# alexfreudenberg/miraculix

Measured on AMD Instinct MI355X. Metric: effective GFLOP/s for dgemm_compressed (2-bit SNP x fp64), higher is better.
Workload: dtype f64; 1 GPU; 1000000x50000 (SNPs x indiv), ncol=32, dgemm_compressed N+T per step, uncentred; snps=1000000, indiv=50000, ncol=32, parallelism=snp-shard1, form=one process per GPU

## Files before the change

include/miraculix_amd.h:

```cpp
#ifndef MIRACULIX_AMD_H
#define MIRACULIX_AMD_H

#include <stdbool.h>
#include <stddef.h>
#include <stdint.h>

#ifdef __cplusplus
extern "C" {
#endif
#if defined(__GNUC__)
#pragma GCC visibility push(default)
#endif


void setOptions_compressed(int use_gpu, int cores, int floatLoop, int meanSubstract, int ignore_missings,
                           int do_not_center, int do_normalize, int use_miraculix_freq, int variant,
                           int print_details);

void plink2compressed(char *plink, char *plink_transposed, int snps, int indiv, double *f, int max_n,
                      void **compressed);

void dgemm_compressed(char *trans, void *compressed, int n, double *B, int Ldb, double *C, int Ldc);

void free_compressed(void **compressed);
// ... 62 lines not shown
} mxa_multi_info;
typedef struct mxa_shard_info {
  int device; long snp_begin, snp_end;
  int peer_to_root, peer_from_root;
  int kernel_launches; double kernel_ms;
  int in_copies; double in_ms;
  int out_copies; double out_ms;
  int pushes; double push_ms;
} mxa_shard_info;
int mxa_multi_get_info(void *compressed, mxa_multi_info *out);
int mxa_multi_shard_info(void *compressed, int shard, mxa_shard_info *out);
int mxa_multi_reset_profile(void *compressed);

int mxa_snp_multiply_panel(const unsigned char *snp_matrix, int snps, int indiv, int col_begin, int col_end, int upper_only,
                           double *panel, long ld, int is_plink_format);

int mxa_grm(const unsigned char *plink_transposed, int snps, int indiv, double *G, int is_plink_format, int do_scale,
            const double *allele_freq);
int mxa_ld(const unsigned char *plink, int snps, int indiv, double *R, int is_plink_format, const double *allele_freq);

int mxa_ld_band(const unsigned char *plink, int snps, int indiv, int window, double *band, long ldb, int kind, int is_plink_format,
                const double *allele_freq);
int mxa_ld_scores(const unsigned char *plink, int snps, int indiv, int window, double *scores, int adjust, int is_plink_format,
                  const double *allele_freq);

int mxa_ld_band_pairwise(const unsigned char *plink, int snps, int indiv, int window, double *band, long ldb, int kind);
int mxa_ld_scores_pairwise(const unsigned char *plink, int snps, int indiv, int window, double *scores, int adjust);

int mxa_set_engine(int engine);
int mxa_get_engine(void);
int mxa_last_path(void);
int mxa_last_range_fallback(void *compressed);

void mxa_profile_reset(void);
void mxa_profile_get(int *launches, double *total_ms);

void mxa_last_geometry(long *m, long *k, int *n, int *splits, int *a_tile, int *c_tile);
long mxa_plan_partial_doubles(long m, long k, int n);
int mxa_single_orientation(void *compressed);
long mxa_partial_capacity(void *compressed);

#if defined(__GNUC__)
#pragma GCC visibility pop
#endif
#ifdef __cplusplus
}
#endif
#endif
```

miraculix_amd/csrc/mxa_api.cpp:

```cpp
#include "../../include/miraculix_amd.h"
#include "mxa_internal.h"

#include <algorithm>
#include <atomic>
#include <chrono>
#include <cstdarg>
#include <cstdio>
#include <cstdlib>
#include <cstring>
#include <mutex>
#include <string>
#include <vector>

namespace mxa {

static int g_err = 0;
static char g_errmsg[512] = "";

Options &options() { static Options o; return o; }
Profile &profile() { static Profile p; return p; }
Geometry &last_geometry() { static Geometry g; return g; }
static bool g_profile_on = true;
static std::atomic<int> g_engine{[] {
  const char *e = getenv("MXA_ENGINE");
// ... 695 lines not shown
  const bool use_lut = n <= 2 && !no_plain;
  GemmPlan p = use_lut ? plan_lut(m, G.k_pad, n) : plan_gemm(m, G.k_pad, n);
  int splits_per_group = p.splits;
  if (!use_lut) {
    const size_t one = (size_t)p.n_pad * p.m_pad, need = one * p.splits;
    const size_t budget = partial_budget(w, need, one);
    if (budget < need) {
      splits_per_group = (int)std::max<size_t>(1, budget / one);
      GemmPlan pg = p; pg.splits = splits_per_group;
      if (ensure_partials(w, pg, s)) return 1;
    }
  }
  if (splits_per_group == p.splits && ensure_partials(w, p, s)) return 1;
  clock_mark("partials");
  {
    std::lock_guard<std::mutex> lk(g_prof_mutex);
    Geometry &geo = last_geometry();
    geo.m = m; geo.k = k; geo.n = n; geo.splits = p.splits; geo.a = p.a; geo.c = p.c; geo.path = use_lut ? 1 : 0;
  }
  const bool tr = !use_lut && gemm_use_tr(p, h, trans);
  const PackedMatrix &GL = gemm_operand(h, trans, tr);
  int mode = gemm_default_mode(p.c);
  const int *d_E = nullptr;
  if (!use_lut && (mode == 2 || mode == 3)) {
    if (w.cap_exp < (size_t)n) {
      MXA_HIP(hipStreamSynchronize(s));
      if (w.d_exp) { MXA_HIP(hipFree(w.d_exp)); w.d_exp = nullptr; w.cap_exp = 0; }
      MXA_HIP(hipMalloc(reinterpret_cast<void **>(&w.d_exp), sizeof(int) * (size_t)n));
      w.cap_exp = n;
    }
    if (launch_colexp(dB, ldb, k, n, w.d_colpart, w.d_exp, 0, s, w.d_denflag, kDenMaxSpan, -100000)) return 1;
    d_E = w.d_exp;
  }
  if (!use_lut && launch_pack_B(dB, ldb, k, n, w.d_Bp, G.k_pad, p.n_pad, p.c, s, d_E, 0, -1, nullptr, mode == 3 && !tr)) return 1;
  if (prof) MXA_HIP(hipEventRecord(pe0, s));
  if (splits_per_group < p.splits) {
    const size_t stride = (size_t)p.n_pad * p.m_pad;
    for (int pass = 0; pass < (d_E ? 2 : 1); pass++) {
      const int *gate = pass ? w.d_denflag : nullptr;
      if (pass && launch_pack_B(dB, ldb, k, n, w.d_Bp, G.k_pad, p.n_pad, p.c, s, nullptr, 0, -1, gate)) return 1;
      for (int sb = 0; sb < p.splits; sb += splits_per_group) {
        const int se = std::min(p.splits, sb + splits_per_group);
        if ((size_t)(se - sb) * stride > w.cap_P) { set_error(4, "internal: a group of %d K splits exceeds the partial-sum workspace", se - sb); return 1; }
        if (launch_gemm(GL, w.d_Bp, w.d_P, p, pass ? 0 : mode, s, next_ctr(w), sb, se, gate, tr, sb)) return 1;
        const int group = (sb > 0 ? 1 : 0) | (se < p.splits ? 2 : 0);
        if (launch_finish(w.d_P, p, m, n, dC, ldc, fill_rows, trans ? 1 : 0, centered, d_sumB, d_sumfB, h->d_f, s, pass ? nullptr : d_E, 0, 0, gate, nullptr, se - sb, group)) return 1;
      }
      if (!pass && prof) { MXA_HIP(hipEventRecord(pe1, s)); h->prof_pending[slot] = true; }
    }
    return 0;
  }
  int rc = use_lut ? launch_lut(G, dB, ldb, n, w.d_P, p, s) : launch_gemm(GL, w.d_Bp, w.d_P, p, mode, s, next_ctr(w), 0, -1, nullptr, tr);
  if (prof && !rc) { MXA_HIP(hipEventRecord(pe1, s)); h->prof_pending[slot] = true; }
  if (!rc && d_E) {
    rc = launch_pack_B(dB, ldb, k, n, w.d_Bp, G.k_pad, p.n_pad, p.c, s, nullptr, 0, -1, w.d_denflag);
    if (!rc) rc = launch_gemm(GL, w.d_Bp, w.d_P, p, 0, s, next_ctr(w), 0, -1, w.d_denflag, tr);
  }
  if (!rc) rc = launch_finish(w.d_P, p, m, n, dC, ldc, fill_rows, trans ? 1 : 0, centered, d_sumB, d_sumfB, h->d_f, s, d_E, 0, 0, nullptr, d_E ? w.d_denflag : nullptr);
  return rc;
}


constexpr int kPipeChunks = 8;
static const size_t kPipeMinBytes = (size_t)32 << 20;

static int pipe_setup(Handle *h) {
  for (hipStream_t &ps : h->pipe) if (!ps) MXA_HIP(hipStreamCreateWithFlags(&ps, hipStreamNonBlocking));
  for (hipEvent_t &e : h->pev) if (!e) MXA_HIP(hipEventCreateWithFlags(&e, hipEventDisableTiming));
  return 0;
}

static int gemm_host_pipelined(Handle *h, bool trans, int n, const double *B, long ldb, bool b_host, bool b_local, double *C, long ldc, bool c_host, bool c_local,
                               long fill_rows) {
  const int engine = g_engine.load();
  if ((engine != 0 && engine != 3) || n < 3 || getenv("MXA_DIAG")) return 2;
  if (engine == 0 && n <= kSmallNMaxColsHost) return 2;
  const PackedMatrix &G = trans ? h->snp_major : h->ind_major;
  const long m = G.rows, k = G.k;
  const size_t b_bytes = b_host ? sizeof(double) * (size_t)k * n : 0, c_bytes = c_host ? sizeof(double) * (size_t)m * n : 0;
  if (std::max(b_bytes, c_bytes) < kPipeMinBytes) return 2;
  const bool kmode = b_bytes >= c_bytes;
  const bool centered = options().centered;
  if (centered && !h->has_f) { set_error(6, "dgemm_compressed: centring requested but no allele frequencies were supplied to plink2compressed"); return 1; }
  if (n > h->max_n) h->max_n = n;
  if (ensure_workspace(h, n) || pipe_setup(h)) return 1;
  harvest_profile(h);
  Workspace &w = h->ws;
  hipStream_t s = h->stream;
  if (grow(&w.d_colpart, &w.cap_colpart, (size_t)n * (128 * (kPipeChunks + 1) + 2) + 16)) return 1;
// ... 501 lines not shown
int mxa_set_engine(int engine) {
  if (engine != 0 && engine != 1 && engine != 3 && engine != 4) return g_engine.load();
  return g_engine.exchange(engine);
}
int mxa_get_engine(void) { return g_engine.load(); }

void mxa_profile_reset(void) { profile() = Profile(); }
void mxa_profile_get(int *launches, double *total_ms) {
  if (launches) *launches = profile().launches;
  if (total_ms) *total_ms = profile().total_ms;
}
int mxa_last_path(void) {
  Geometry g;
  { std::lock_guard<std::mutex> lk(g_prof_mutex); g = last_geometry(); }
  if (g.path != 4) return g.path;
  int flag = 0, prev = 0;
  if (!g.d_flag) return 2;
  (void)hipGetDevice(&prev);
  if (hipSetDevice(g.flag_dev) != hipSuccess || hipMemcpy(&flag, g.d_flag, sizeof(int), hipMemcpyDeviceToHost) != hipSuccess) { (void)hipGetLastError(); flag = 0; }
  (void)hipSetDevice(prev);
  return flag ? 3 : 2;
}
int mxa_last_range_fallback(void *compressed) {
  if (!compressed || is_multi(compressed)) return -1;
  Handle *h = as_handle(compressed, "mxa_last_range_fallback");
  if (!h || !h->ws.d_denflag) return -1;
  int flag = 0, prev = 0;
  (void)hipGetDevice(&prev);
  if (hipSetDevice(h->device) != hipSuccess || hipStreamSynchronize(h->stream) != hipSuccess ||
      hipMemcpy(&flag, h->ws.d_denflag, sizeof(int), hipMemcpyDeviceToHost) != hipSuccess) { (void)hipGetLastError(); flag = -1; }
  (void)hipSetDevice(prev);
  return flag;
}
void mxa_last_geometry(long *m, long *k, int *n, int *splits, int *a_tile, int *c_tile) {
  const Geometry &g = last_geometry();
  if (m) *m = g.m; if (k) *k = g.k; if (n) *n = g.n; if (splits) *splits = g.splits; if (a_tile) *a_tile = g.a; if (c_tile) *c_tile = g.c;
}

long mxa_plan_partial_doubles(long m, long k, int n) {
  if (m <= 0 || k <= 0 || n <= 0) return 0;
  const GemmPlan p = plan_gemm(m, (k + kSlabK - 1) / kSlabK * kSlabK, n);
  return (long)p.splits * p.n_pad * p.m_pad;
}
int mxa_single_orientation(void *compressed) {
  if (!compressed) return -1;
  if (is_multi(compressed)) return multi_single(compressed);
  Handle *h = as_handle(compressed, "mxa_single_orientation");
  return h ? (h->single ? 1 : 0) : -1;
}
long mxa_partial_capacity(void *compressed) {
  if (!compressed || is_multi(compressed)) return -1;
  Handle *h = as_handle(compressed, "mxa_partial_capacity");
  return h ? (long)h->ws.cap_P : -1;
}

static long count_lines(const char *path) {
  FILE *fh = fopen(path, "rb");
  if (!fh) return -1;
  long n = 0; int c, last = '\n';
  while ((c = fgetc(fh)) != EOF) { if (c == '\n') n++; last = c; }
  if (last != '\n') n++;
  fclose(fh);
  return n;
}

static std::string bed_base(const char *bed_path) {
// ... 198 lines not shown
```

miraculix_amd/csrc/mxa_internal.h:

```cpp
#pragma once
#include <hip/hip_runtime.h>
#include <cstddef>
#include <cstdint>
#include <functional>
#include <utility>
#include <vector>
#include "mxa_plan.h"

namespace mxa {

constexpr int kWaves = 4;
constexpr int kKStep = 16;
constexpr int kSlabSteps = 8;
constexpr int kSlabK = kKStep * kSlabSteps;
constexpr int kSlabBytes = kSlabK / 4;
constexpr int kRowAlign = 512;
constexpr int kTileRows = 256;
constexpr int kTileBytes = kTileRows * kSlabBytes;

struct Options {
  bool gpu = true;
  bool centered = true;
  int print_level = 0;
  bool set = false;
// ... 100 lines not shown
int bed_range_to_handle(const char *base, long snps_total, long indiv, long snp_begin, long snp_end, int max_n, int device, void **out,
                        double *f_out_local);
constexpr int kMaxShards = 64;
struct PartList { const double *p[kMaxShards]; int count; };
int launch_reduce_parts(const PartList &parts, long m, int n, double *dC, long ldc, long fill_rows, hipStream_t s);

void set_error(int code, const char *fmt, ...);
void clear_error();
bool check_hip(hipError_t e, const char *func, int line);
#define MXA_HIP(x) do { if (!::mxa::check_hip((x), __func__, __LINE__)) return 1; } while (0)
void debug_info(const char *fmt, ...);
struct CallClock {
  bool on = false;
  double t0 = 0.0, last = 0.0;
  char line[512]; int len = 0;
  static double now();
  void start(bool enabled) { on = enabled; len = 0; line[0] = 0; if (on) t0 = last = now(); }
  void mark(const char *what);
  void report(const char *head);
};
extern thread_local CallClock *tl_call_clock;
inline void clock_mark(const char *what) { if (tl_call_clock && tl_call_clock->on) tl_call_clock->mark(what); }

int launch_recode(const uint8_t *d_src, size_t src_pitch, long row0, long nrows, long k, long k_bit_offset,
                  PackedMatrix &dst, hipStream_t s);
constexpr int kDenUp = 900;
constexpr int kDenMaxSpan = 800;
constexpr int kI8ExactMaxDigits = 24;
int launch_colspan(const double *dB, long ldb, long k, int n, double *d_part, int *d_out3, hipStream_t s);
int launch_colexp_from_part(const double *d_part, int n, int *d_E, int bias, hipStream_t s);
int launch_colexp(const double *dB, long ldb, long k, int n, double *d_part, int *d_E, int bias, hipStream_t s, int *d_flag = nullptr, int max_span = 0,
                  int min_emax = 0, bool reset_flag = true);
int launch_pack_B(const double *dB, long ldb, long k, int n, double *dBp, long k_pad, int n_pad, int c, hipStream_t s, const int *d_E = nullptr, long S0 = 0,
                  long S_cnt = -1, const int *run_if_set = nullptr, bool rowscale = false);
int launch_colsums(const double *dB, long ldb, long k, int n, const double *d_f , double *d_part,
                   double *d_sumB, double *d_sumfB, hipStream_t s);
GemmPlan plan_gemm(long m, long k_pad, int n, const GemmPlan *ksplits_like = nullptr);
int gemm_default_mode(int c);
int launch_gemm(const PackedMatrix &G, const double *dBp, double *dP, const GemmPlan &p, int mode, hipStream_t s, int *d_ctr, int split_begin = 0, int split_end = -1,
                const int *run_if_set = nullptr, bool tr = false, int p_split0 = 0);
GemmPlan plan_lut(long m, long k_pad, int n);
int launch_lut(const PackedMatrix &G, const double *dB, long ldb, int n, double *dP, const GemmPlan &p, hipStream_t s, const int *run_if_set = nullptr);
int launch_finish(const double *dP, const GemmPlan &p, long m, int n, double *dC, long ldc, long fill_rows, int mode_trans,
                  bool centered, const double *d_sumB, const double *d_sumfB, const double *d_f, hipStream_t s, const int *d_E = nullptr, int e_splits = 0,
                  int e_stride = 0, const int *run_if_set = nullptr, const int *unscaled_if_set = nullptr, int group_splits = 0, int group = 0);
int ensure_dyn_lds(const void *func, int bytes, unsigned long long *mask);
int launch_transpose_2bit(const uint8_t *d_in, long rows, long cols, uint8_t *d_out, hipStream_t s);
int launch_allele_freq(const uint8_t *d_plink, long snps, long indiv, double *d_f, hipStream_t s);
int launch_plink_lut(uint8_t *d, size_t nbytes, hipStream_t s);
int launch_sparse_times_plink(const uint8_t *dP, size_t pitch, long entries, int nIdx, const int *d_rowIdx, const int *d_colIdx, const double *d_val,
                              double *dC_slab, long ldc, long e_base, long e_count, hipStream_t s);
struct I8Chain { int S0 = 0, S1 = 0, my_class = 0; bool first = true; bool fp64_rows = true; };
int gemm_i8_device(const PackedMatrix &G, bool trans, int n, const double *dB, long ldb, double *dC, long ldc, long fill_rows, bool centered, double *d_sumB,
                   double *d_sumfB, const double *d_f, Workspace &w, hipStream_t s, hipEvent_t ev0, hipEvent_t ev1, int *splits_out, int guard = 0,
                   const int **flag_out = nullptr, double *colsum_scratch = nullptr, int S_override = 0, const PackedMatrix *G_tn = nullptr,
                   double *stats_part = nullptr, const I8Chain *chain = nullptr);
int gemm_i8_reserve(const PackedMatrix &G, int n, int S, const PackedMatrix *G_tn, Workspace &w, hipStream_t s);

int launch_dgemm(bool ta, bool tb, long M, long N, long K, double alpha, const double *A, long lda, const double *B, long ldb, double beta, double *C, long ldc,
                 bool lower_only, hipStream_t s);
int launch_potrf_inv_block(double *A, long ld, int nb, long offset, int *info, double *inv_out, hipStream_t s);

}
```

miraculix_amd/csrc/mxa_kernels.hip:

```cpp
#include "mxa_internal.h"
#include "mxa_queue.h"
#include <algorithm>
#include <cstdio>
#include <cstdlib>
#include <vector>

namespace mxa {

constexpr long kMaxBlocksPerLaunch = 1L << 23;

__device__ __forceinline__ uint32_t recode16(uint32_t w) {
  const uint32_t H = (w >> 1) & 0x55555555u, L = w & 0x55555555u;
  return ((H & L) << 1) | (H & ~L);
}

__global__ void __launch_bounds__(256) k_recode(const uint8_t *__restrict__ src, size_t src_pitch, long src_row_bytes,
                                                long nrows, long k, uint8_t *__restrict__ dst, long dst_row0, long nslabs, long rows_blocks, long blk0) {
  const long bid = blk0 + blockIdx.x;
  const long rblk = bid % rows_blocks, sgrp = bid / rows_blocks;
  const int rr = threadIdx.x >> 3, part = threadIdx.x & 7;
  const long r = rblk * 32 + rr;
  const long slab = sgrp * 4 + (part >> 1);
  if (r >= nrows || slab >= nslabs) return;
  const long b = slab * kSlabBytes + (part & 1) * 16;
// ... 26 lines not shown
  const long grid = rows_blocks * slab_groups;
  for (long b0 = 0; b0 < grid; b0 += kMaxBlocksPerLaunch) {
    const long nb = std::min(kMaxBlocksPerLaunch, grid - b0);
    hipLaunchKernelGGL(k_recode, dim3((unsigned)nb), dim3(256), 0, s, d_src, src_pitch, (k + 3) / 4, nrows, k, dst.d, row0, dst.nslabs, rows_blocks, b0);
  }
  MXA_HIP(hipGetLastError());
  return 0;
}

__host__ __device__ __forceinline__ long gemm_k_index(long S, int kk) { return (S >> 3) * 128 + 16 * (kk & 7) + 8 * (kk >> 3) + (S & 7); }

__global__ void __launch_bounds__(256) k_pack_B(const double *__restrict__ B, long ldb, long k, int n,
                                                double *__restrict__ Bp, long total, int C, long S_total, const int *__restrict__ E, int up, long S0, long S_cnt,
                                                const int *__restrict__ run_if_set, int rowscale) {
  if (run_if_set && *run_if_set == 0) return;
  for (long idx = (long)blockIdx.x * blockDim.x + threadIdx.x; idx < total; idx += (long)gridDim.x * blockDim.x) {
    const int l = (int)(idx & 63);
    const long sh = idx >> 6;
    const int h = (int)(sh % C);
    const long cs = sh / C;
    const long S = S0 + cs % S_cnt;
    const int chunk = (int)(cs / S_cnt);
    const long row = gemm_k_index(S, l >> 2);
    const int col = chunk * 4 * C + 4 * h + (l & 3);
    double v = 0.0;
    if (row < k && col < n) {
      v = B[row + (long)col * ldb];
      if (E) v = ldexp(v, up - E[col] - (rowscale ? 2 * (int)(row & 15) : 0));
    }
    Bp[(((size_t)chunk * S_total + S) * C + h) * 64 + l] = v;
  }
}

__global__ void __launch_bounds__(256) k_colmax_partial(const double *__restrict__ B, long ldb, long k, double *__restrict__ part, int n, int want_min) {
  const int j = blockIdx.y, c = blockIdx.x;
  const long per = (k + 63) / 64;
  const long c0 = c * per, c1 = std::min<long>(k, c0 + per);
  const double inf = __longlong_as_double(0x7ff0000000000000ll);
  double m = 0.0, lo = inf;
  for (long r = c0 + threadIdx.x; r < c1; r += 256) {
    const double a = fabs(B[r + (long)j * ldb]);
    m = (a <= 1.7976931348623157e308) ? fmax(m, a) : inf;
    if (a > 0.0) lo = fmin(lo, a);
  }
  __shared__ double sh[256], sl[256];
  sh[threadIdx.x] = m; sl[threadIdx.x] = lo;
  __syncthreads();
  for (int w = 128; w > 0; w >>= 1) {
    if ((int)threadIdx.x < w) { sh[threadIdx.x] = fmax(sh[threadIdx.x], sh[threadIdx.x + w]); sl[threadIdx.x] = fmin(sl[threadIdx.x], sl[threadIdx.x + w]); }
    __syncthreads();
  }
  if (threadIdx.x == 0) { part[(size_t)j * 64 + c] = sh[0]; if (want_min) part[((size_t)n + j) * 64 + c] = sl[0]; }
}
__global__ void k_colexp_final(const double *__restrict__ part, int n, int bias, int *__restrict__ E, int *__restrict__ flag, int max_span, int min_emax) {
  const int j = blockIdx.x * blockDim.x + threadIdx.x;
  if (j >= n) return;
  double m = 0.0;
  for (int c = 0; c < 64; c++) m = fmax(m, part[(size_t)j * 64 + c]);
  int e = 0;
  if (m > 0.0 && isfinite(m)) (void)frexp(m, &e);
  E[j] = e + bias;
  if (flag) {
    bool ok = isfinite(m);
    if (ok && m > 0.0) {
      double lo = m;
      for (int c = 0; c < 64; c++) lo = fmin(lo, part[((size_t)n + j) * 64 + c]);
      int el = 0;
      (void)frexp(lo, &el);
      ok = e >= min_emax && el >= e - max_span;
    }
    if (!ok) atomicOr(flag, 1);
  }
}
int launch_colexp(const double *dB, long ldb, long k, int n, double *d_part, int *d_E, int bias, hipStream_t s, int *d_flag, int max_span, int min_emax, bool reset_flag) {
  if (d_flag && reset_flag) MXA_HIP(hipMemsetAsync(d_flag, 0, sizeof(int), s));
  hipLaunchKernelGGL(k_colmax_partial, dim3(64, n), dim3(256), 0, s, dB, ldb, k, d_part, n, d_flag ? 1 : 0);
  hipLaunchKernelGGL(k_colexp_final, dim3((n + 63) / 64), dim3(64), 0, s, d_part, n, bias, d_E, d_flag, max_span, min_emax);
  MXA_HIP(hipGetLastError());
  return 0;
}

int launch_colexp_from_part(const double *d_part, int n, int *d_E, int bias, hipStream_t s) {
  hipLaunchKernelGGL(k_colexp_final, dim3((n + 63) / 64), dim3(64), 0, s, d_part, n, bias, d_E, (int *)nullptr, 0, 0);
  MXA_HIP(hipGetLastError());
  return 0;
}

__global__ void __launch_bounds__(256) k_colspan_final(const double *__restrict__ part, int n, int *__restrict__ out) {
  __shared__ int s_span[256], s_emax[256], s_bad[256];
  int span = 0, emin_max = 1 << 20, bad = 0;
  for (int j = threadIdx.x; j < n; j += 256) {
    double m = 0.0;
    for (int c = 0; c < 64; c++) m = fmax(m, part[(size_t)j * 64 + c]);
    if (!isfinite(m)) { bad = 1; continue; }
    if (m > 0.0) {
      double lo = m;
      for (int c = 0; c < 64; c++) lo = fmin(lo, part[((size_t)n + j) * 64 + c]);
      int e = 0, el = 0;
      (void)frexp(m, &e); (void)frexp(lo, &el);
      span = max(span, e - el); emin_max = min(emin_max, e);
    }
  }
  s_span[threadIdx.x] = span; s_emax[threadIdx.x] = emin_max; s_bad[threadIdx.x] = bad;
  __syncthreads();
  for (int w = 128; w > 0; w >>= 1) {
    if ((int)threadIdx.x < w) {
      s_span[threadIdx.x] = max(s_span[threadIdx.x], s_span[threadIdx.x + w]); s_emax[threadIdx.x] = min(s_emax[threadIdx.x], s_emax[threadIdx.x + w]);
      s_bad[threadIdx.x] |= s_bad[threadIdx.x + w];
    }
    __syncthreads();
  }
  if (threadIdx.x == 0) { out[0] = s_span[0]; out[1] = s_emax[0] == (1 << 20) ? 0 : s_emax[0]; out[2] = s_bad[0]; }
}
int launch_colspan(const double *dB, long ldb, long k, int n, double *d_part, int *d_out3, hipStream_t s) {
  hipLaunchKernelGGL(k_colmax_partial, dim3(64, n), dim3(256), 0, s, dB, ldb, k, d_part, n, 1);
  hipLaunchKernelGGL(k_colspan_final, dim3(1), dim3(256), 0, s, d_part, n, d_out3);
  MXA_HIP(hipGetLastError());
  return 0;
}

int launch_pack_B(const double *dB, long ldb, long k, int n, double *dBp, long k_pad, int n_pad, int c, hipStream_t s, const int *d_E, long S0, long S_cnt,
                  const int *run_if_set, bool rowscale) {
  const long S_total = k_pad / 16;
  if (S_cnt < 0) S_cnt = S_total - S0;
  const long total = S_cnt * (long)(n_pad / 4) * 64;
  if (total <= 0) return 0;
  const int grid = (int)std::min<long>((total + 255) / 256, 256L * 64);
  hipLaunchKernelGGL(k_pack_B, dim3(grid), dim3(256), 0, s, dB, ldb, k, n, dBp, total, c, S_total, d_E, kDenUp, S0, S_cnt, run_if_set, rowscale ? 1 : 0);
  MXA_HIP(hipGetLastError());
  return 0;
}

constexpr int kColChunks = 64;

__global__ void __launch_bounds__(256) k_colsum_partial(const double *__restrict__ B, long ldb, long k,
                                                        const double *__restrict__ f, double *__restrict__ part) {
  const int j = blockIdx.y, c = blockIdx.x;
  const long per = (k + kColChunks - 1) / kColChunks;
  const long c0 = c * per, c1 = std::min<long>(k, c0 + per);
  double s1 = 0.0, s2 = 0.0;
  for (long r = c0 + threadIdx.x; r < c1; r += 256) {
    const double b = B[r + (long)j * ldb];
    s1 += b;
    if (f) s2 = fma(f[r], b, s2);
  }
  __shared__ double sh1[256], sh2[256];
  sh1[threadIdx.x] = s1; sh2[threadIdx.x] = s2;
  __syncthreads();
  for (int w = 128; w > 0; w >>= 1) {
    if ((int)threadIdx.x < w) { sh1[threadIdx.x] += sh1[threadIdx.x + w]; sh2[threadIdx.x] += sh2[threadIdx.x + w]; }
    __syncthreads();
  }
  if (threadIdx.x == 0) {
    part[((size_t)j * kColChunks + c) * 2 + 0] = sh1[0];
    part[((size_t)j * kColChunks + c) * 2 + 1] = sh2[0];
  }
}

// ... 267 lines not shown
      }
      asm volatile("s_waitcnt lgkmcnt(0)" ::: "memory");
      __builtin_amdgcn_wave_barrier();
    }
    if (DIAG && threadIdx.x == 0 && diag) {
      diag[2 * (size_t)bid] = t1 - t0; diag[2 * (size_t)bid + 1] = r1 - r0;
      diag[2 * (size_t)nunits + 2 * (size_t)bid] = rt_begin; diag[2 * (size_t)nunits + 2 * (size_t)bid + 1] = r0;
      diag[4 * (size_t)nunits + bid] = __builtin_amdgcn_s_memrealtime();
    }
    if (next < 0) break;
    u = un; bid = next;
    asm volatile("s_waitcnt vmcnt(0)" ::: "memory");
    __syncthreads();
  }
}

int gemm_default_mode(int) {
  return 3;
}

static long device_cus() {
  static const long r = [] {
    int dev = 0; hipDeviceProp_t prop;
    if (hipGetDevice(&dev) != hipSuccess || hipGetDeviceProperties(&prop, dev) != hipSuccess) { (void)hipGetLastError(); return 256L; }
    return (long)prop.multiProcessorCount;
  }();
  return r > 0 ? r : 256;
}

GemmPlan plan_gemm(long m, long k_pad, int n, const GemmPlan *ksplits_like) { return plan_gemm_host(m, k_pad, n, device_cus(), ksplits_like); }

template <int A, int C, int MODE, bool TR = false>
static int launch_gemm_t(const PackedMatrix &G, const double *dBp, double *dP, const GemmPlan &p, hipStream_t s, int split_begin, int split_end, const int *run_if_set,
                         int *d_ctr, int p_split0) {
  using Cfg = GemmCfg<A, C>;
  static unsigned long long attr_mask = 0;
  if (ensure_dyn_lds(reinterpret_cast<const void *>(&k_gemm<A, C, MODE, false, TR>), Cfg::kLds, &attr_mask)) return 1;
  const long nunits = (long)p.rowblocks * p.nchunks * (split_end - split_begin);
  if (nunits > 0x3fffffffL) { set_error(3, "launch too large"); return 1; }
  if (nunits <= 0) return 0;
  if (!d_ctr) { set_error(4, "internal: k_gemm needs its queue counters"); return 1; }
  static int per_cu[64] = {};
  int dev = 0;
  MXA_HIP(hipGetDevice(&dev));
  if (!per_cu[dev & 63]) {
    int nb = 0;
    MXA_HIP(hipOccupancyMaxActiveBlocksPerMultiprocessor(&nb, reinterpret_cast<const void *>(&k_gemm<A, C, MODE, false, TR>), 256, Cfg::kLds));
    hipDeviceProp_t prop;
    MXA_HIP(hipGetDeviceProperties(&prop, dev));
    per_cu[dev & 63] = std::max(1, std::min(nb, gemm_wg_per_cu(C))) * prop.multiProcessorCount;
  }
  const long grid = std::min<long>(nunits, per_cu[dev & 63]);
  constexpr int xcd_order = 1;
  const KSplit ks{p.s1, p.l1, p.r1, p.l2};
  const int long_groups = (std::min(split_end, p.s1) - std::min(split_begin, p.s1)) * p.nchunks;
  const int g8 = xcd_order ? (long_groups & ~7) : 0;
  MXA_HIP(hipMemsetAsync(d_ctr, 0, 9 * sizeof(int), s));
  static const bool diag_on = getenv("MXA_DIAG") != nullptr;
  if (!TR && diag_on && ((A == 8 && C == 8) || (A == 16 && C == 1)) && split_begin == 0 && split_end == p.splits && !run_if_set) {
    static unsigned long long attr2 = 0;
    if (ensure_dyn_lds(reinterpret_cast<const void *>(&k_gemm<A, C, MODE, true>), Cfg::kLds, &attr2)) return 1;
    unsigned long long *d_diag = nullptr;
    MXA_HIP(hipMalloc(reinterpret_cast<void **>(&d_diag), sizeof(unsigned long long) * 5 * nunits));
    MXA_HIP(hipMemsetAsync(d_diag, 0, sizeof(unsigned long long) * 5 * nunits, s));
    hipLaunchKernelGGL((k_gemm<A, C, MODE, true>), dim3((unsigned)grid), dim3(256), Cfg::kLds, s, G.d, G.pitch, dBp, p.n_pad / 4, dP,
                       p.m_pad, p.n_pad, p.rowblocks, p.nchunks, p.slabs_total, ks, xcd_order, d_diag, split_begin, (const int *)nullptr, (int)nunits, d_ctr, g8, p_split0);
    MXA_HIP(hipStreamSynchronize(s));
    std::vector<unsigned long long> h(5 * nunits);
    MXA_HIP(hipMemcpy(h.data(), d_diag, sizeof(unsigned long long) * 5 * nunits, hipMemcpyDeviceToHost));
    std::vector<double> ghz, cyc;
    for (long i = 0; i < nunits; i++) if (h[2 * i + 1]) {
      const int sp = (int)(i < (long)g8 * p.rowblocks ? ((i & 7) + 8 * ((i >> 3) / p.rowblocks)) / p.nchunks : (i / p.rowblocks) / p.nchunks);
      const int len = ksplit_len(ks, sp);
      ghz.push_back((double)h[2 * i] / (double)h[2 * i + 1] * 0.1); cyc.push_back((double)h[2 * i] / len);
    }
    std::sort(ghz.begin(), ghz.end()); std::sort(cyc.begin(), cyc.end());
    if (!ghz.empty()) printf("MXA_DIAG k_gemm<%d,%d,%d>: %ld pieces on %ld workgroups (splits %d = %d x %d + short x %d), in-kernel clock median %.3f GHz (min %.3f max %.3f); shader cycles per slab median %.0f (ideal %d)\n",
                             A, C, MODE, nunits, grid, p.splits, p.s1, p.l1, p.l2, ghz[ghz.size() / 2], ghz.front(), ghz.back(), cyc[cyc.size() / 2], kSlabSteps * A * C * 16 * 2);
    double ticks = 0.0;
    for (long i = 0; i < nunits; i++) ticks += (double)h[2 * i + 1];
    printf("MXA_DIAG k_gemm: K loops of all pieces = %.3f ms if packed perfectly on %ld resident slots (compare with the kernel duration)\n", ticks * 1e-5 / (double)grid, grid);
    {
      double life = 0; unsigned long long first = ~0ull, last = 0;
      for (long i = 0; i < nunits; i++) {
        const unsigned long long b = h[2 * nunits + 2 * i], e = h[4 * nunits + i];
        life += (double)(e - b);
        first = std::min(first, b); last = std::max(last, e);
      }
      printf("MXA_DIAG k_gemm: mean piece lifetime %.1f us; span first begin -> last end %.3f ms; sum of lifetimes / slots = %.3f ms\n",
             life / nunits * 1e-2, (double)(last - first) * 1e-5, life * 1e-5 / (double)grid);
      std::vector<std::pair<unsigned long long, int>> ev;
      ev.reserve(2 * nunits);
      for (long i = 0; i < nunits; i++) { ev.emplace_back(h[2 * nunits + 2 * i], +1); ev.emplace_back(h[4 * nunits + i], -1); }
      std::sort(ev.begin(), ev.end());
      const unsigned long long win = 200000;
      double idle[3] = {0, 0, 0}; long active = 0, max_active = 0; unsigned long long prev_t = first;
      for (auto &e : ev) {
        unsigned long long t0 = prev_t, t1 = e.first;
        while (t0 < t1) {
          const int zone = t0 < first + win ? 0 : (t0 >= last - win ? 2 : 1);
          const unsigned long long border = zone == 0 ? first + win : (zone == 1 ? last - win : last);
          const unsigned long long te = std::min(t1, std::max(border, t0 + 1));
          idle[zone] += (double)(te - t0) * (double)(grid - std::min(active, grid));
          t0 = te;
        }
        active += e.second; max_active = std::max(max_active, active); prev_t = e.first;
      }
      printf("MXA_DIAG k_gemm: idle slot-time first 2 ms %.3f ms, middle %.3f ms, last 2 ms %.3f ms; max pieces in flight %ld\n",
             idle[0] * 1e-5 / (double)grid, idle[1] * 1e-5 / (double)grid, idle[2] * 1e-5 / (double)grid, max_active);
    }
    (void)hipFree(d_diag);
    return 0;
  }
  hipLaunchKernelGGL((k_gemm<A, C, MODE, false, TR>), dim3((unsigned)grid), dim3(256), Cfg::kLds, s, G.d, G.pitch, dBp, p.n_pad / 4, dP,
                     p.m_pad, p.n_pad, p.rowblocks, p.nchunks, p.slabs_total, ks, xcd_order, (unsigned long long *)nullptr, split_begin, run_if_set, (int)nunits, d_ctr, g8, p_split0);
  MXA_HIP(hipGetLastError());
  return 0;
}

int launch_gemm(const PackedMatrix &G, const double *dBp, double *dP, const GemmPlan &p, int mode, hipStream_t s, int *d_ctr, int split_begin, int split_end,
                const int *run_if_set, bool tr, int p_split0) {
  if (split_end < 0) split_end = p.splits;
  if (p_split0 < 0 || p_split0 > split_begin) { set_error(4, "internal: k_gemm partial-sum base split %d outside [0, %d]", p_split0, split_begin); return 1; }
  if (!G.d) { set_error(4, "internal: k_gemm was given a packed matrix that is not stored (single-orientation object)"); return 1; }
  if (tr) {
    if ((long)p.slabs_total * kSlabK > G.rows_pad || G.nslabs < 1 || (mode != 0 && mode != 3)) {
      set_error(4, "internal: transposed launch does not fit the packed matrix (K slabs %d x 128 > %ld rows) or mode %d", p.slabs_total, G.rows_pad, mode);
      return 1;
    }
#define MXA_DISPATCH_TR(AA, CC)                                                                                          \
    if (p.a == AA && p.c == CC) {                                                                                        \
      if (mode == 3) return launch_gemm_t<AA, CC, 3, true>(G, dBp, dP, p, s, split_begin, split_end, nullptr, d_ctr, p_split0);     \
      return launch_gemm_t<AA, CC, 0, true>(G, dBp, dP, p, s, split_begin, split_end, run_if_set, d_ctr, p_split0);                 \
    }
    MXA_DISPATCH_TR(16, 1) MXA_DISPATCH_TR(16, 2) MXA_DISPATCH_TR(16, 3) MXA_DISPATCH_TR(16, 4)
    MXA_DISPATCH_TR(8, 5) MXA_DISPATCH_TR(8, 6) MXA_DISPATCH_TR(8, 7) MXA_DISPATCH_TR(8, 8)
#undef MXA_DISPATCH_TR
    set_error(5, "internal: no transposed kernel for tile a=%d c=%d", p.a, p.c);
    return 1;
  }
  if (p.m_pad > G.rows_pad || (size_t)p.slabs_total * kSlabBytes > G.pitch) {
    set_error(4, "internal: packed matrix smaller than the launch plan (m_pad %ld > %ld or k bytes %ld > pitch %zu)", p.m_pad,
              G.rows_pad, (long)p.slabs_total * kSlabBytes, G.pitch);
    return 1;
  }
#define MXA_DISPATCH(AA, CC)                                              \
  if (p.a == AA && p.c == CC) {                                           \
    if (mode == 3) return launch_gemm_t<AA, CC, 3>(G, dBp, dP, p, s, split_begin, split_end, nullptr, d_ctr, p_split0);     \
    return launch_gemm_t<AA, CC, 0>(G, dBp, dP, p, s, split_begin, split_end, run_if_set, d_ctr, p_split0);                 \
  }
  MXA_DISPATCH(16, 1)
  MXA_DISPATCH(16, 2)
  MXA_DISPATCH(16, 3)
  MXA_DISPATCH(16, 4)
  MXA_DISPATCH(8, 5)
  MXA_DISPATCH(8, 6)
  MXA_DISPATCH(8, 7)
  MXA_DISPATCH(8, 8)
#undef MXA_DISPATCH
  set_error(5, "internal: no kernel for tile a=%d c=%d", p.a, p.c);
  return 1;
}

template <int NV, int KS, int WV>
struct LutCfg {
  static constexpr int kThreads = 64 * WV;
  static constexpr int kRows = kThreads;
  static constexpr int kChunks = KS / 64;
  static constexpr int kRowBytes = kRows * KS / 4;
  static constexpr int kTabBytes = (KS / 2) * 16 * 8 * NV;
  static constexpr int kBufBytes = kRowBytes + kTabBytes;
  static constexpr int kLds = 2 * kBufBytes;
};

template <int NV, int KS, int WV>
__global__ void __launch_bounds__(64 * WV)
k_lut(const uint8_t *__restrict__ G, size_t pitch, const double *__restrict__ B, long ldb, long k, int n, double *__restrict__ P,
      long m_pad, int rowblocks, int slabs_total, int slabs_per_split, const int *__restrict__ run_if_set) {
  using Cfg = LutCfg<NV, KS, WV>;
  extern __shared__ __attribute__((aligned(16))) char smem[];
  if (run_if_set && *run_if_set == 0) return;
  const int tid = threadIdx.x, lane = tid & 63;
// ... 401 lines not shown
```

miraculix_amd/lib.py:

```python
import ctypes
import os

_HERE = os.path.dirname(os.path.abspath(__file__))
_DEFAULT = os.path.join(_HERE, "lib", "libmiraculix_amd.so")
_LIBRARY_PATH = [os.environ.get("MIRACULIX_AMD_LIBRARY", _DEFAULT)]
_LIBRARY_HANDLE = [None]

c_u8p = ctypes.POINTER(ctypes.c_uint8)
c_f64p = ctypes.POINTER(ctypes.c_double)


class MultiInfo(ctypes.Structure):
    _fields_ = [("shards", ctypes.c_int), ("devices", ctypes.c_int), ("root_device", ctypes.c_int), ("reduction", ctypes.c_int),
                ("reductions", ctypes.c_int), ("reduce_ms", ctypes.c_double), ("rccl_checked", ctypes.c_int), ("rccl_vs_p2p_max_rel_diff", ctypes.c_double)]


class ShardInfo(ctypes.Structure):
    _fields_ = [("device", ctypes.c_int), ("snp_begin", ctypes.c_long), ("snp_end", ctypes.c_long), ("peer_to_root", ctypes.c_int), ("peer_from_root", ctypes.c_int),
                ("kernel_launches", ctypes.c_int), ("kernel_ms", ctypes.c_double), ("in_copies", ctypes.c_int), ("in_ms", ctypes.c_double),
                ("out_copies", ctypes.c_int), ("out_ms", ctypes.c_double), ("pushes", ctypes.c_int), ("push_ms", ctypes.c_double)]


def set_library_path(path):
    _LIBRARY_PATH[0] = path
# ... 78 lines not shown
    L.mxa_gram_matvec.argtypes = [ctypes.c_void_p, ctypes.c_int, ctypes.c_void_p, ctypes.c_long, ctypes.c_void_p, ctypes.c_long]
    L.mxa_gram_matvec.restype = ctypes.c_int
    L.mxa_gram_matvec_device.argtypes = [ctypes.c_void_p, ctypes.c_int, ctypes.c_void_p, ctypes.c_long, ctypes.c_void_p, ctypes.c_long, ctypes.c_int]
    L.mxa_gram_matvec_device.restype = ctypes.c_int
    L.mxa_snp_multiply_panel.argtypes = [ctypes.c_void_p, ctypes.c_int, ctypes.c_int, ctypes.c_int, ctypes.c_int, ctypes.c_int, ctypes.c_void_p, ctypes.c_long, ctypes.c_int]
    L.mxa_snp_multiply_panel.restype = ctypes.c_int
    L.potrs_solve_gpu.argtypes = [ctypes.c_void_p, ctypes.c_uint, ctypes.c_void_p, ctypes.c_uint, ctypes.c_void_p, ctypes.c_void_p, ctypes.c_int, ctypes.POINTER(ctypes.c_int)]
    L.potrs_solve_gpu.restype = None
    L.potrs_solve.argtypes = [ctypes.c_void_p, ctypes.c_uint, ctypes.c_void_p, ctypes.c_uint, ctypes.c_void_p, ctypes.c_void_p, ctypes.c_int]
    L.potrs_solve.restype = ctypes.c_int
    L.sparse2gpu.argtypes = [ctypes.c_void_p, ctypes.c_void_p, ctypes.c_void_p, ctypes.c_long, ctypes.c_long, ctypes.c_long, ctypes.c_int, ctypes.POINTER(ctypes.c_void_p), ctypes.POINTER(ctypes.c_int)]
    L.sparse2gpu.restype = None
    L.dcsrtrsv_solve_gpu.argtypes = [ctypes.c_void_p, ctypes.c_char, ctypes.c_void_p, ctypes.c_long, ctypes.c_void_p, ctypes.POINTER(ctypes.c_int)]
    L.dcsrtrsv_solve_gpu.restype = None
    L.free_sparse_gpu.argtypes = [ctypes.POINTER(ctypes.c_void_p), ctypes.POINTER(ctypes.c_int)]
    L.free_sparse_gpu.restype = None
    L.mxa_set_engine.argtypes = [ctypes.c_int]
    L.mxa_set_engine.restype = ctypes.c_int
    L.mxa_get_engine.restype = ctypes.c_int
    L.mxa_last_path.restype = ctypes.c_int
    L.mxa_last_range_fallback.argtypes = [ctypes.c_void_p]
    L.mxa_last_range_fallback.restype = ctypes.c_int
    L.mxa_profile_reset.restype = None
    L.mxa_profile_get.argtypes = [ctypes.POINTER(ctypes.c_int), ctypes.POINTER(ctypes.c_double)]
    L.mxa_profile_get.restype = None
    L.mxa_last_geometry.argtypes = [ctypes.POINTER(ctypes.c_long), ctypes.POINTER(ctypes.c_long), ctypes.POINTER(ctypes.c_int), ctypes.POINTER(ctypes.c_int), ctypes.POINTER(ctypes.c_int), ctypes.POINTER(ctypes.c_int)]
    L.mxa_last_geometry.restype = None
    L.mxa_single_orientation.argtypes = [ctypes.c_void_p]
    L.mxa_single_orientation.restype = ctypes.c_int
    L.mxa_partial_capacity.argtypes = [ctypes.c_void_p]
    L.mxa_partial_capacity.restype = ctypes.c_long
    L.mxa_plan_partial_doubles.argtypes = [ctypes.c_long, ctypes.c_long, ctypes.c_int]
    L.mxa_plan_partial_doubles.restype = ctypes.c_long
    _LIBRARY_HANDLE[0] = L
    return L


def check_library_handle():
    if _LIBRARY_HANDLE[0] is None:
        load_shared_library()
    return _LIBRARY_HANDLE[0]


def last_error():
    L = check_library_handle()
    return L.mxa_last_error(), (L.mxa_last_error_string() or b"").decode()


def is_torch_tensor(x):
    return type(x).__module__.startswith("torch")


def ptr(x):
    if x is None:
        return None
    if is_torch_tensor(x):
        return ctypes.c_void_p(x.data_ptr())
    return ctypes.c_void_p(x.ctypes.data)
```

Measured before the change: 74520 GFLOP/s.

## Tile B packing through LDS, vectorize column-max scan, fold memsets into kernels

```diff
diff --git a/include/miraculix_amd.h b/include/miraculix_amd.h
--- a/include/miraculix_amd.h
+++ b/include/miraculix_amd.h
@@ -118,6 +118,9 @@
 int mxa_last_path(void);
 int mxa_last_range_fallback(void *compressed);
 
+int mxa_test_prepare_B(const double *dB, long ldb, long k, int n, double *d_part, int *d_E, int *d_flag, double *dBp, long k_pad, int c, int rowscale,
+                       long S0, long S_cnt);
+
 void mxa_profile_reset(void);
 void mxa_profile_get(int *launches, double *total_ms);
 
diff --git a/miraculix_amd/csrc/mxa_api.cpp b/miraculix_amd/csrc/mxa_api.cpp
--- a/miraculix_amd/csrc/mxa_api.cpp
+++ b/miraculix_amd/csrc/mxa_api.cpp
@@ -751,7 +751,8 @@
     if (launch_colexp(dB, ldb, k, n, w.d_colpart, w.d_exp, 0, s, w.d_denflag, kDenMaxSpan, -100000)) return 1;
     d_E = w.d_exp;
   }
-  if (!use_lut && launch_pack_B(dB, ldb, k, n, w.d_Bp, G.k_pad, p.n_pad, p.c, s, d_E, 0, -1, nullptr, mode == 3 && !tr)) return 1;
+  int *const ctr_main = !use_lut && splits_per_group == p.splits ? next_ctr(w) : nullptr;
+  if (!use_lut && launch_pack_B(dB, ldb, k, n, w.d_Bp, G.k_pad, p.n_pad, p.c, s, d_E, 0, -1, nullptr, mode == 3 && !tr, ctr_main)) return 1;
   if (prof) MXA_HIP(hipEventRecord(pe0, s));
   if (splits_per_group < p.splits) {
     const size_t stride = (size_t)p.n_pad * p.m_pad;
@@ -769,11 +770,12 @@
     }
     return 0;
   }
-  int rc = use_lut ? launch_lut(G, dB, ldb, n, w.d_P, p, s) : launch_gemm(GL, w.d_Bp, w.d_P, p, mode, s, next_ctr(w), 0, -1, nullptr, tr);
+  int rc = use_lut ? launch_lut(G, dB, ldb, n, w.d_P, p, s) : launch_gemm(GL, w.d_Bp, w.d_P, p, mode, s, ctr_main, 0, -1, nullptr, tr, 0, true);
   if (prof && !rc) { MXA_HIP(hipEventRecord(pe1, s)); h->prof_pending[slot] = true; }
   if (!rc && d_E) {
-    rc = launch_pack_B(dB, ldb, k, n, w.d_Bp, G.k_pad, p.n_pad, p.c, s, nullptr, 0, -1, w.d_denflag);
-    if (!rc) rc = launch_gemm(GL, w.d_Bp, w.d_P, p, 0, s, next_ctr(w), 0, -1, w.d_denflag, tr);
+    int *const ctr_fb = next_ctr(w);
+    rc = launch_pack_B(dB, ldb, k, n, w.d_Bp, G.k_pad, p.n_pad, p.c, s, nullptr, 0, -1, w.d_denflag, false, ctr_fb);
+    if (!rc) rc = launch_gemm(GL, w.d_Bp, w.d_P, p, 0, s, ctr_fb, 0, -1, w.d_denflag, tr, 0, true);
   }
   if (!rc) rc = launch_finish(w.d_P, p, m, n, dC, ldc, fill_rows, trans ? 1 : 0, centered, d_sumB, d_sumfB, h->d_f, s, d_E, 0, 0, nullptr, d_E ? w.d_denflag : nullptr);
   return rc;
@@ -1341,6 +1343,14 @@
   (void)hipSetDevice(prev);
   return flag;
 }
+int mxa_test_prepare_B(const double *dB, long ldb, long k, int n, double *d_part, int *d_E, int *d_flag, double *dBp, long k_pad, int c, int rowscale, long S0, long S_cnt) {
+  if (!dB || !d_part || !d_E || !dBp || k <= 0 || n <= 0 || ldb < k || k_pad < k || k_pad % kSlabK != 0 || c < 1 || c > 8 || (n + 4 * c - 1) / (4 * c) > 1024) return 1;
+  const int n_pad = (n + 4 * c - 1) / (4 * c) * 4 * c;
+  if (S0 < 0 || S0 > k_pad / 16 || (S_cnt >= 0 && S0 + S_cnt > k_pad / 16)) return 1;
+  if (launch_colexp(dB, ldb, k, n, d_part, d_E, 0, nullptr, d_flag, kDenMaxSpan, -100000)) return 1;
+  if (launch_pack_B(dB, ldb, k, n, dBp, k_pad, n_pad, c, nullptr, d_E, S0, S_cnt, nullptr, rowscale != 0)) return 1;
+  return check_hip(hipStreamSynchronize(nullptr), __func__, __LINE__) ? 0 : 1;
+}
 void mxa_last_geometry(long *m, long *k, int *n, int *splits, int *a_tile, int *c_tile) {
   const Geometry &g = last_geometry();
   if (m) *m = g.m; if (k) *k = g.k; if (n) *n = g.n; if (splits) *splits = g.splits; if (a_tile) *a_tile = g.a; if (c_tile) *c_tile = g.c;
diff --git a/miraculix_amd/csrc/mxa_internal.h b/miraculix_amd/csrc/mxa_internal.h
--- a/miraculix_amd/csrc/mxa_internal.h
+++ b/miraculix_amd/csrc/mxa_internal.h
@@ -156,13 +156,15 @@
 int launch_colexp(const double *dB, long ldb, long k, int n, double *d_part, int *d_E, int bias, hipStream_t s, int *d_flag = nullptr, int max_span = 0,
                   int min_emax = 0, bool reset_flag = true);
 int launch_pack_B(const double *dB, long ldb, long k, int n, double *dBp, long k_pad, int n_pad, int c, hipStream_t s, const int *d_E = nullptr, long S0 = 0,
-                  long S_cnt = -1, const int *run_if_set = nullptr, bool rowscale = false);
+                  long S_cnt = -1, const int *run_if_set = nullptr, bool rowscale = false, int *zero_ctr = nullptr);
+constexpr int kGemmCtrInts = 9;
+bool gemm_prep_tiled();
 int launch_colsums(const double *dB, long ldb, long k, int n, const double *d_f , double *d_part,
                    double *d_sumB, double *d_sumfB, hipStream_t s);
 GemmPlan plan_gemm(long m, long k_pad, int n, const GemmPlan *ksplits_like = nullptr);
 int gemm_default_mode(int c);
 int launch_gemm(const PackedMatrix &G, const double *dBp, double *dP, const GemmPlan &p, int mode, hipStream_t s, int *d_ctr, int split_begin = 0, int split_end = -1,
-                const int *run_if_set = nullptr, bool tr = false, int p_split0 = 0);
+                const int *run_if_set = nullptr, bool tr = false, int p_split0 = 0, bool ctr_zeroed = false);
 GemmPlan plan_lut(long m, long k_pad, int n);
 int launch_lut(const PackedMatrix &G, const double *dB, long ldb, int n, double *dP, const GemmPlan &p, hipStream_t s, const int *run_if_set = nullptr);
 int launch_finish(const double *dP, const GemmPlan &p, long m, int n, double *dC, long ldc, long fill_rows, int mode_trans,
diff --git a/miraculix_amd/csrc/mxa_kernels.hip b/miraculix_amd/csrc/mxa_kernels.hip
--- a/miraculix_amd/csrc/mxa_kernels.hip
+++ b/miraculix_amd/csrc/mxa_kernels.hip
@@ -82,6 +82,43 @@
   }
 }
 
+constexpr int kPackTileStride = 144;
+__global__ void __launch_bounds__(256) k_pack_B_tiled(const double *__restrict__ B, long ldb, long k, int n, double *__restrict__ Bp, int C, long S_total,
+                                                      const int *__restrict__ E, int up, long slab0, long nslabs, long ntiles, const int *__restrict__ run_if_set,
+                                                      int rowscale, int *__restrict__ zero_ints, int zero_cnt) {
+  if (zero_ints && blockIdx.x == 0 && (int)threadIdx.x < zero_cnt) zero_ints[threadIdx.x] = 0;
+  if (run_if_set && *run_if_set == 0) return;
+  __shared__ double tile[32 * kPackTileStride];
+  const int elems = C * 512;
+  for (long tix = blockIdx.x; tix < ntiles; tix += gridDim.x) {
+    const long chunk = tix / nslabs, slab = slab0 + (tix - chunk * nslabs);
+    const long row0 = slab * 128;
+    const int col0 = (int)chunk * 4 * C;
+#pragma unroll 4
+    for (int e = threadIdx.x; e < elems; e += 256) {
+      const int cl = e >> 7, r = e & 127, col = col0 + cl;
+      const long row = row0 + r;
+      double v = 0.0;
+      if (row < k && col < n) {
+        v = B[row + (long)col * ldb];
+        if (E) v = ldexp(v, up - E[col] - (rowscale ? 2 * (r & 15) : 0));
+      }
+      tile[cl * kPackTileStride + (r ^ (r >> 4))] = v;
+    }
+    __syncthreads();
+    double *__restrict__ out = Bp + ((size_t)chunk * S_total + (size_t)slab * 8) * C * 64;
+    const int l = threadIdx.x & 63, kk = l >> 2, rl = 16 * (kk & 7) + 8 * (kk >> 3);
+    int h = threadIdx.x >> 6, t = 0;
+    for (int run = threadIdx.x >> 6; run < 8 * C; run += 4) {
+      while (h >= C) { h -= C; t++; }
+      const int r = rl + t;
+      out[run * 64 + l] = tile[(4 * h + (l & 3)) * kPackTileStride + (r ^ (r >> 4))];
+      h += 4;
+    }
+    __syncthreads();
+  }
+}
+
 __global__ void __launch_bounds__(256) k_colmax_partial(const double *__restrict__ B, long ldb, long k, double *__restrict__ part, int n, int want_min) {
   const int j = blockIdx.y, c = blockIdx.x;
   const long per = (k + 63) / 64;
@@ -92,6 +129,45 @@
     const double a = fabs(B[r + (long)j * ldb]);
     m = (a <= 1.7976931348623157e308) ? fmax(m, a) : inf;
     if (a > 0.0) lo = fmin(lo, a);
+  }
+  __shared__ double sh[256], sl[256];
+  sh[threadIdx.x] = m; sl[threadIdx.x] = lo;
+  __syncthreads();
+  for (int w = 128; w > 0; w >>= 1) {
+    if ((int)threadIdx.x < w) { sh[threadIdx.x] = fmax(sh[threadIdx.x], sh[threadIdx.x + w]); sl[threadIdx.x] = fmin(sl[threadIdx.x], sl[threadIdx.x + w]); }
+    __syncthreads();
+  }
+  if (threadIdx.x == 0) { part[(size_t)j * 64 + c] = sh[0]; if (want_min) part[((size_t)n + j) * 64 + c] = sl[0]; }
+}
+__device__ __forceinline__ void colmax_take(double a, double &m, double &lo, double inf) {
+  a = fabs(a);
+  m = (a <= 1.7976931348623157e308) ? fmax(m, a) : inf;
+  if (a > 0.0) lo = fmin(lo, a);
+}
+__global__ void __launch_bounds__(256) k_colmax_partial_wide(const double *__restrict__ B, long ldb, long k, double *__restrict__ part, int n, int want_min,
+                                                             int *__restrict__ zero_flag) {
+  const int j = blockIdx.y, c = blockIdx.x;
+  if (zero_flag && j == 0 && c == 0 && threadIdx.x == 0) *zero_flag = 0;
+  const long per = (k + 63) / 64;
+  const long c0 = c * per, c1 = std::min<long>(k, c0 + per);
+  const double inf = __longlong_as_double(0x7ff0000000000000ll);
+  double m = 0.0, lo = inf;
+  if (c0 < c1) {
+    const double *col = B + (long)j * ldb;
+    const long head = (long)((reinterpret_cast<size_t>(col + c0) >> 3) & 1);
+    const long pairs = (c1 - c0 - head) / 2;
+    const double2 *__restrict__ p2 = reinterpret_cast<const double2 *>(col + c0 + head);
+    if (threadIdx.x == 0 && head) colmax_take(col[c0], m, lo, inf);
+    if (threadIdx.x == 1 && c0 + head + 2 * pairs < c1) colmax_take(col[c1 - 1], m, lo, inf);
+    long i = threadIdx.x;
+    for (; i + 7 * 256 < pairs; i += 8 * 256) {
+      double2 v[8];
+#pragma unroll
+      for (int u = 0; u < 8; u++) v[u] = p2[i + u * 256];
+#pragma unroll
+      for (int u = 0; u < 8; u++) { colmax_take(v[u].x, m, lo, inf); colmax_take(v[u].y, m, lo, inf); }
+    }
+    for (; i < pairs; i += 256) { const double2 v = p2[i]; colmax_take(v.x, m, lo, inf); colmax_take(v.y, m, lo, inf); }
   }
   __shared__ double sh[256], sl[256];
   sh[threadIdx.x] = m; sl[threadIdx.x] = lo;
@@ -122,9 +198,14 @@
     if (!ok) atomicOr(flag, 1);
   }
 }
+bool gemm_prep_tiled() { const char *e = getenv("MXA_GEMM_PREP"); return !(e && e[0] == '0'); }
 int launch_colexp(const double *dB, long ldb, long k, int n, double *d_part, int *d_E, int bias, hipStream_t s, int *d_flag, int max_span, int min_emax, bool reset_flag) {
-  if (d_flag && reset_flag) MXA_HIP(hipMemsetAsync(d_flag, 0, sizeof(int), s));
-  hipLaunchKernelGGL(k_colmax_partial, dim3(64, n), dim3(256), 0, s, dB, ldb, k, d_part, n, d_flag ? 1 : 0);
+  if (gemm_prep_tiled()) {
+    hipLaunchKernelGGL(k_colmax_partial_wide, dim3(64, n), dim3(256), 0, s, dB, ldb, k, d_part, n, d_flag ? 1 : 0, reset_flag ? d_flag : (int *)nullptr);
+  } else {
+    if (d_flag && reset_flag) MXA_HIP(hipMemsetAsync(d_flag, 0, sizeof(int), s));
+    hipLaunchKernelGGL(k_colmax_partial, dim3(64, n), dim3(256), 0, s, dB, ldb, k, d_part, n, d_flag ? 1 : 0);
+  }
   hipLaunchKernelGGL(k_colexp_final, dim3((n + 63) / 64), dim3(64), 0, s, d_part, n, bias, d_E, d_flag, max_span, min_emax);
   MXA_HIP(hipGetLastError());
   return 0;
@@ -163,17 +244,27 @@
   if (threadIdx.x == 0) { out[0] = s_span[0]; out[1] = s_emax[0] == (1 << 20) ? 0 : s_emax[0]; out[2] = s_bad[0]; }
 }
 int launch_colspan(const double *dB, long ldb, long k, int n, double *d_part, int *d_out3, hipStream_t s) {
-  hipLaunchKernelGGL(k_colmax_partial, dim3(64, n), dim3(256), 0, s, dB, ldb, k, d_part, n, 1);
+  if (gemm_prep_tiled()) hipLaunchKernelGGL(k_colmax_partial_wide, dim3(64, n), dim3(256), 0, s, dB, ldb, k, d_part, n, 1, (int *)nullptr);
+  else hipLaunchKernelGGL(k_colmax_partial, dim3(64, n), dim3(256), 0, s, dB, ldb, k, d_part, n, 1);
   hipLaunchKernelGGL(k_colspan_final, dim3(1), dim3(256), 0, s, d_part, n, d_out3);
   MXA_HIP(hipGetLastError());
   return 0;
 }
 
 int launch_pack_B(const double *dB, long ldb, long k, int n, double *dBp, long k_pad, int n_pad, int c, hipStream_t s, const int *d_E, long S0, long S_cnt,
-                  const int *run_if_set, bool rowscale) {
+                  const int *run_if_set, bool rowscale, int *zero_ctr) {
   const long S_total = k_pad / 16;
   if (S_cnt < 0) S_cnt = S_total - S0;
   const long total = S_cnt * (long)(n_pad / 4) * 64;
+  if (total > 0 && gemm_prep_tiled() && S0 % kSlabSteps == 0 && S_cnt % kSlabSteps == 0 && c >= 1 && c <= 8 && n_pad % (4 * c) == 0) {
+    const long nslabs = S_cnt / kSlabSteps, ntiles = nslabs * (n_pad / (4 * c));
+    const int grid = (int)std::min<long>(ntiles, 2048);
+    hipLaunchKernelGGL(k_pack_B_tiled, dim3(grid), dim3(256), 0, s, dB, ldb, k, n, dBp, c, S_total, d_E, kDenUp, S0 / kSlabSteps, nslabs, ntiles, run_if_set,
+                       rowscale ? 1 : 0, zero_ctr, kGemmCtrInts);
+    MXA_HIP(hipGetLastError());
+    return 0;
+  }
+  if (zero_ctr) MXA_HIP(hipMemsetAsync(zero_ctr, 0, kGemmCtrInts * sizeof(int), s));
   if (total <= 0) return 0;
   const int grid = (int)std::min<long>((total + 255) / 256, 256L * 64);
   hipLaunchKernelGGL(k_pack_B, dim3(grid), dim3(256), 0, s, dB, ldb, k, n, dBp, total, c, S_total, d_E, kDenUp, S0, S_cnt, run_if_set, rowscale ? 1 : 0);
@@ -507,7 +598,7 @@
 
 template <int A, int C, int MODE, bool TR = false>
 static int launch_gemm_t(const PackedMatrix &G, const double *dBp, double *dP, const GemmPlan &p, hipStream_t s, int split_begin, int split_end, const int *run_if_set,
-                         int *d_ctr, int p_split0) {
+                         int *d_ctr, int p_split0, bool ctr_zeroed) {
   using Cfg = GemmCfg<A, C>;
   static unsigned long long attr_mask = 0;
   if (ensure_dyn_lds(reinterpret_cast<const void *>(&k_gemm<A, C, MODE, false, TR>), Cfg::kLds, &attr_mask)) return 1;
@@ -530,7 +621,7 @@
   const KSplit ks{p.s1, p.l1, p.r1, p.l2};
   const int long_groups = (std::min(split_end, p.s1) - std::min(split_begin, p.s1)) * p.nchunks;
   const int g8 = xcd_order ? (long_groups & ~7) : 0;
-  MXA_HIP(hipMemsetAsync(d_ctr, 0, 9 * sizeof(int), s));
+  if (!ctr_zeroed) MXA_HIP(hipMemsetAsync(d_ctr, 0, kGemmCtrInts * sizeof(int), s));
   static const bool diag_on = getenv("MXA_DIAG") != nullptr;
   if (!TR && diag_on && ((A == 8 && C == 8) || (A == 16 && C == 1)) && split_begin == 0 && split_end == p.splits && !run_if_set) {
     static unsigned long long attr2 = 0;
@@ -594,7 +685,7 @@
 }
 
 int launch_gemm(const PackedMatrix &G, const double *dBp, double *dP, const GemmPlan &p, int mode, hipStream_t s, int *d_ctr, int split_begin, int split_end,
-                const int *run_if_set, bool tr, int p_split0) {
+                const int *run_if_set, bool tr, int p_split0, bool ctr_zeroed) {
   if (split_end < 0) split_end = p.splits;
   if (p_split0 < 0 || p_split0 > split_begin) { set_error(4, "internal: k_gemm partial-sum base split %d outside [0, %d]", p_split0, split_begin); return 1; }
   if (!G.d) { set_error(4, "internal: k_gemm was given a packed matrix that is not stored (single-orientation object)"); return 1; }
@@ -605,8 +696,8 @@
     }
 #define MXA_DISPATCH_TR(AA, CC)                                                                                          \
     if (p.a == AA && p.c == CC) {                                                                                        \
-      if (mode == 3) return launch_gemm_t<AA, CC, 3, true>(G, dBp, dP, p, s, split_begin, split_end, nullptr, d_ctr, p_split0);     \
-      return launch_gemm_t<AA, CC, 0, true>(G, dBp, dP, p, s, split_begin, split_end, run_if_set, d_ctr, p_split0);                 \
+      if (mode == 3) return launch_gemm_t<AA, CC, 3, true>(G, dBp, dP, p, s, split_begin, split_end, nullptr, d_ctr, p_split0, ctr_zeroed);     \
+      return launch_gemm_t<AA, CC, 0, true>(G, dBp, dP, p, s, split_begin, split_end, run_if_set, d_ctr, p_split0, ctr_zeroed);                 \
     }
     MXA_DISPATCH_TR(16, 1) MXA_DISPATCH_TR(16, 2) MXA_DISPATCH_TR(16, 3) MXA_DISPATCH_TR(16, 4)
     MXA_DISPATCH_TR(8, 5) MXA_DISPATCH_TR(8, 6) MXA_DISPATCH_TR(8, 7) MXA_DISPATCH_TR(8, 8)
@@ -621,8 +712,8 @@
   }
 #define MXA_DISPATCH(AA, CC)                                              \
   if (p.a == AA && p.c == CC) {                                           \
-    if (mode == 3) return launch_gemm_t<AA, CC, 3>(G, dBp, dP, p, s, split_begin, split_end, nullptr, d_ctr, p_split0);     \
-    return launch_gemm_t<AA, CC, 0>(G, dBp, dP, p, s, split_begin, split_end, run_if_set, d_ctr, p_split0);                 \
+    if (mode == 3) return launch_gemm_t<AA, CC, 3>(G, dBp, dP, p, s, split_begin, split_end, nullptr, d_ctr, p_split0, ctr_zeroed);     \
+    return launch_gemm_t<AA, CC, 0>(G, dBp, dP, p, s, split_begin, split_end, run_if_set, d_ctr, p_split0, ctr_zeroed);                 \
   }
   MXA_DISPATCH(16, 1)
   MXA_DISPATCH(16, 2)
diff --git a/miraculix_amd/lib.py b/miraculix_amd/lib.py
--- a/miraculix_amd/lib.py
+++ b/miraculix_amd/lib.py
@@ -134,6 +134,9 @@
     L.mxa_partial_capacity.restype = ctypes.c_long
     L.mxa_plan_partial_doubles.argtypes = [ctypes.c_long, ctypes.c_long, ctypes.c_int]
     L.mxa_plan_partial_doubles.restype = ctypes.c_long
+    L.mxa_test_prepare_B.argtypes = [ctypes.c_void_p, ctypes.c_long, ctypes.c_long, ctypes.c_int, ctypes.c_void_p, ctypes.c_void_p, ctypes.c_void_p, ctypes.c_void_p, ctypes.c_long,
+                                     ctypes.c_int, ctypes.c_int, ctypes.c_long, ctypes.c_long]
+    L.mxa_test_prepare_B.restype = ctypes.c_int
     _LIBRARY_HANDLE[0] = L
     return L
 
```

Result: no change. 74600 GFLOP/s (median of 6 runs) (+0.1%).
